# facebookresearch/PoseDiffusion

Hardware: AMD Instinct MI355X
Metric: sequences/sec (20-frame, GGS on) (higher is better)
Workload: dtype f32 (GGS, attention, LayerNorm, DDPM update, every accumulation); the encoder GEMMs multiply fp16 hi + lo operand pairs (22 bits, static power-of-two scales) with fp32 accumulation -- `exact_mode` is the same pipe with them on the exact-fp32 matrix instruction

## Files before the change

### posediffusion_amd/csrc/pd_denoiser.hip

```cpp
#include "pd_denoiser_dev.h"
#include "pd_gemm_stream.h"
#include "pd_gemm_split.h"
#include "pd_qkv_attn.h"
#ifndef PD_STRIP_RT3
#define PD_STRIP_RT3 1
#endif
#ifndef PD_STRIP_RT1
#define PD_STRIP_RT1 0
#endif
#ifndef PD_STRIP_RT3_FF1
#define PD_STRIP_RT3_FF1 0
#endif
#ifndef PD_STRIP_K64
#define PD_STRIP_K64 true
#endif

#include <algorithm>
#include <math.h>
#include <stdlib.h>
#include <string.h>

__global__ __launch_bounds__(256) void pd_embed_rows_kernel(const float *__restrict__ x, int n_frames, int M, float *__restrict__ out) {
    const int row = blockIdx.x * 4 + (threadIdx.x >> 6), lane = threadIdx.x & 63;
    if (row >= M) return;
// ... 571 lines not shown
static size_t attn_seq_lds(int N) { return ((size_t)3 * N * (DH + 4) + 4 * PD_ATTN_RPW * 64) * sizeof(float); }

struct HeadArgs {
    const float *hid;
    const float *lnw, *lnb, *w3, *b3;
    const float *x;
    const float *noise;
    float *eps_out, *mean_out, *x0_out, *xnext_out;
    float c_recip, c_recipm1, coef1, coef2, sigma;
    int M;
    int pred_x0;
#ifdef PD_DEN_STAMPS
    long long *stamps;
#endif
};

__global__ __launch_bounds__(256) void pd_tail_kernel(HeadArgs g) {
#ifdef PD_DEN_STAMPS
    long long *const stamps = g.stamps;
#endif
    PD_STAMP(stamps, 0);
    const int lane = threadIdx.x & 63, wave = threadIdx.x >> 6;
    const int m = blockIdx.x * 4 + wave;
    if (m >= g.M) return;
    const float *row = g.hid + (size_t)m * HID;
    const float v0 = row[lane], v1 = row[64 + lane];
    const int l9 = lane < 9 ? lane : 8;
    const size_t at = (size_t)m * 9 + l9;
    const float b3v = g.b3[l9], xv = g.x[at], nz = g.noise ? g.noise[at] : 0.0f;
    const float mean = pd_wave_sum(v0 + v1) * (1.0f / HID);
    const float d0 = v0 - mean, d1 = v1 - mean;
    const float rstd = 1.0f / sqrtf(pd_wave_sum(d0 * d0 + d1 * d1) * (1.0f / HID) + 1e-5f);
    const float a0 = pd_relu(d0 * rstd * g.lnw[lane] + g.lnb[lane]);
    const float a1 = pd_relu(d1 * rstd * g.lnw[64 + lane] + g.lnb[64 + lane]);
    float e = 0.0f;
#pragma unroll
    for (int o = 0; o < 9; ++o) {
        const float part = pd_wave_sum(fmaf(a0, g.w3[o * HID + lane], a1 * g.w3[o * HID + 64 + lane]));
        e = (lane == o) ? part : e;
    }
    if (lane < 9) {
        e += b3v;
        const float x0 = g.pred_x0 ? e : g.c_recip * xv - g.c_recipm1 * e;
        const float mu = g.coef1 * x0 + g.coef2 * xv;
        if (g.eps_out) g.eps_out[at] = e;
        if (g.x0_out) g.x0_out[at] = x0;
        if (g.mean_out) g.mean_out[at] = mu;
        if (g.xnext_out) g.xnext_out[at] = g.noise ? mu + g.sigma * nz : mu;
    }
    PD_STAMP(stamps, 5);
    PD_STAMP_DRAIN();
    PD_STAMP(stamps, 6);
}

int pd_time_table(const pd_weights *w, float *table) {
    if (!w->time_w0 || !w->time_b0 || !w->time_w2 || !w->time_b2) {
        pd_set_error("pd_engine_create: a weight pointer is NULL");
        return PD_ERR_INVALID_ARG;
    }
    hipLaunchKernelGGL(pd_time_table_kernel, dim3(w->timesteps), dim3(128), 0, 0, w->time_w0, w->time_b0, w->time_w2, w->time_b2, table);
    PD_HIP_CHECK(hipGetLastError());
    return PD_OK;
}

static bool pd_denoiser_default_shape(const pd_weights *w) {
    return w->d_model == DM && w->nhead == NH && w->dim_ff == DFF && w->z_dim == ZD && w->n_harmonic == 10 && w->t_emb_dim == 256 &&
           w->mlp_hidden == HID && w->num_layers >= 1 && w->num_layers <= PD_MAX_LAYERS &&
           !(w->reserved & (PD_WEIGHTS_POST_NORM | PD_WEIGHTS_NO_PIVOT | PD_WEIGHTS_GENERIC));
}

int pd_denoiser_create(pd_engine *eng, const pd_weights *w) {
    if (!pd_denoiser_default_shape(w)) return pd_denoiser_generic_create(eng, w);
    PdDenoiserDev *d = new PdDenoiserDev();
    eng->den = d;
    PdDevAllocs &m = d->mem;
    d->num_layers = w->num_layers;
    d->timesteps = w->timesteps;
    d->m_cap = ((eng->max_B * eng->max_N + 31) / 32) * 32;
    PD_TRY(m.alloc(&d->t_table, (size_t)w->timesteps * 128));
    PD_TRY(pd_time_table(w, d->t_table));
    for (int v = 0; v < 2; ++v) {
        const int nt = v ? 16 : 32;
        PD_TRY(m.pack(&d->first_wp[v], w->first_w, DM, KFIRST, KFIRST_PAD, nt, nullptr, 1));
        PD_TRY(m.pack(&d->last0_wp[v], w->last0_w, HID, DM, DM, nt, nullptr));
        for (int l = 0; l < w->num_layers; ++l) {
            const pd_layer_weights &s = w->layers[l];
            PdLayerDev &L = d->layers[l];
            PD_TRY(m.pack(&L.qkv_wp[v], s.in_proj_w, 3 * DM, DM, DM, nt, s.norm1_w));
            PD_TRY(m.pack(&L.out_wp[v], s.out_proj_w, DM, DM, DM, nt, nullptr));
            PD_TRY(m.pack(&L.ff1_wp[v], s.linear1_w, DFF, DM, DM, nt, s.norm2_w));
            PD_TRY(m.pack(&L.ff2_wp[v], s.linear2_w, DM, DFF, DFF, nt, nullptr));
        }
    }
    PD_TRY(m.copy(&d->first_b, w->first_b, DM));
    for (int l = 0; l < w->num_layers; ++l) {
        const pd_layer_weights &s = w->layers[l];
        PdLayerDev &L = d->layers[l];
        if (!s.norm1_w || !s.norm2_w) {
            pd_set_error("pd_engine_create: a LayerNorm weight pointer is NULL");
            return PD_ERR_INVALID_ARG;
        }
        PD_TRY(m.fold_bias(&L.qkv_b, s.in_proj_w, s.norm1_b, s.in_proj_b, 3 * DM, DM));
        PD_TRY(m.copy(&L.out_b, s.out_proj_b, DM));
        PD_TRY(m.fold_bias(&L.ff1_b, s.linear1_w, s.norm2_b, s.linear1_b, DFF, DM));
        PD_TRY(m.copy(&L.ff2_b, s.linear2_b, DM));
        PD_TRY(m.rowmajor(&L.qkv_wf, s.in_proj_w, 3 * DM, DM, s.norm1_w));
        PD_TRY(m.rowmajor(&L.out_wf, s.out_proj_w, DM, DM, nullptr));
        PD_TRY(m.rowmajor(&L.ff1_wf, s.linear1_w, DFF, DM, s.norm2_w));
        PD_TRY(m.rowmajor(&L.ff2_wf, s.linear2_w, DM, DFF, nullptr));
    }
    PD_TRY(m.copy(&d->last0_b, w->last0_b, HID));
    PD_TRY(m.copy(&d->last_ln_w, w->last_ln_w, HID));
    PD_TRY(m.copy(&d->last_ln_b, w->last_ln_b, HID));
    PD_TRY(m.copy(&d->last3_w, w->last3_w, 9 * HID));
    PD_TRY(m.copy(&d->last3_b, w->last3_b, 9));
    const size_t rows = (size_t)d->m_cap;
    PD_TRY(m.alloc(&d->h, rows * DM));
    PD_TRY(m.alloc(&d->qkv, rows * 3 * DM));
    PD_TRY(m.alloc(&d->ctx, rows * DM));
    PD_TRY(m.alloc(&d->ff, rows * DFF));
    PD_TRY(m.alloc(&d->hid, rows * HID));
    if (rows >= PD_STREAM_MIN_ROWS) PD_TRY(m.alloc(&d->hn, rows * DM));
    if (d->hn) {
        PD_TRY(m.alloc(&d->emb, rows * KFIRST_D));
        PD_TRY(m.alloc(&d->zproj, rows * DM));
        PD_TRY(m.alloc(&d->first_df, (size_t)DM * KFIRST_D));
        PD_TRY(m.alloc(&d->first_zf, (size_t)DM * ZD));
        hipLaunchKernelGGL(pd_first_rowmajor_kernel, dim3((DM * KFIRST_D + 255) / 256), dim3(256), 0, 0, w->first_w, d->first_df, PD_FIRST_D, KFIRST_D);
        hipLaunchKernelGGL(pd_first_rowmajor_kernel, dim3((DM * ZD + 255) / 256), dim3(256), 0, 0, w->first_w, d->first_zf, PD_FIRST_Z, ZD);
        PD_HIP_CHECK(hipGetLastError());
        PD_TRY(m.alloc(&d->ttab, (size_t)w->timesteps * DM));
        hipLaunchKernelGGL(pd_first_ttab_kernel, dim3(w->timesteps), dim3(DM), 0, 0, w->first_w, d->t_table, d->ttab);
        PD_HIP_CHECK(hipGetLastError());
    }
    PD_TRY(m.rowmajor(&d->last0_wf, w->last0_w, HID, DM, nullptr));
    PD_TRY(pd_set_lds(pd_gemm_kernel<KFIRST_PAD, 2, 0, 32>, 32 * (KFIRST_PAD + 4) * 4));
    PD_TRY(pd_set_lds(pd_gemm_kernel<KFIRST_PAD, 2, 0, 16>, 32 * (KFIRST_PAD + 4) * 4));
    PD_TRY(pd_set_lds(pd_gemm_kernel<DM, 1, 0, 32>, 32 * (DM + 4) * 4));
    PD_TRY(pd_set_lds(pd_gemm_kernel<DM, 1, 0, 16>, 32 * (DM + 4) * 4));
    PD_TRY(pd_set_lds(pd_gemm_kernel<DM, 1, 1, 32>, 32 * (DM + 4) * 4));
    PD_TRY(pd_set_lds(pd_gemm_kernel<DM, 1, 1, 16>, 32 * (DM + 4) * 4));
    PD_TRY(pd_set_lds(pd_gemm_kernel<DM, 0, 2, 32>, 32 * (DM + 4) * 4));
    PD_TRY(pd_set_lds(pd_gemm_kernel<DM, 0, 2, 16>, 32 * (DM + 4) * 4));
    PD_TRY(pd_set_lds(pd_gemm_kernel<DFF, 0, 2, 32>, 32 * (DFF + 4) * 4));
    PD_TRY(pd_set_lds(pd_gemm_kernel<DFF, 0, 2, 16>, 32 * (DFF + 4) * 4));
    PD_TRY(pd_set_lds(pd_gemm_kernel<DM, 0, 0, 32>, 32 * (DM + 4) * 4));
    PD_TRY(pd_set_lds(pd_gemm_kernel<DM, 0, 0, 16>, 32 * (DM + 4) * 4));
    PD_TRY(pd_set_lds(pd_attn_kernel<false>, ((2 * 64 + 4) * (DH + 4) + 4 * 64) * 4));
    PD_TRY(pd_set_lds(pd_attn_kernel<true>, ((2 * 64 + 4) * (DH + 4) + 4 * 64) * 4));
    PD_TRY(pd_set_lds(pd_attn_seq_kernel<0>, attn_seq_lds(64)));
    PD_TRY(pd_set_lds(pd_attn_seq_kernel<1>, attn_seq_lds(64)));
    PD_TRY(pd_set_lds(pd_attn_seq_kernel<2>, attn_seq_lds(64)));
    PD_TRY(pd_set_lds(pd_attn_mma_kernel<2>, attn_mma_lds(32)));
    PD_TRY(pd_set_lds((pd_qkv_attn_kernel<0, PD_QA_DEEP_DEFAULT != 0>), 160 * 1024));
#ifdef PD_DEV_KNOBS
    PD_TRY(pd_set_lds((pd_qkv_attn_kernel<0, PD_QA_DEEP_DEFAULT == 0>), 160 * 1024));
    PD_TRY(pd_set_lds(pd_qkv_attn_kernel<1>, 160 * 1024));
    PD_TRY(pd_set_lds(pd_qkv_attn_kernel<2>, 160 * 1024));
    PD_TRY(pd_set_lds(pd_qkv_attn_kernel<3>, 160 * 1024));
    PD_TRY(pd_set_lds(pd_qkv_attn_kernel<4>, 160 * 1024));
    PD_TRY(pd_set_lds(pd_qkv_attn_kernel<5>, 160 * 1024));
#endif
    PD_HIP_CHECK(hipDeviceSynchronize());
    return PD_OK;
}

bool pd_denoiser_has_streamed_path(const pd_engine *eng) { return eng->den && eng->den->hn; }
bool pd_denoiser_weights_non_finite(const pd_engine *eng) { return eng->den && eng->den->non_finite; }

int pd_denoiser_build_split(pd_engine *eng, int mode) {
    if (eng->gden) {
        pd_set_error("split-precision denoiser: this engine runs the shape-generic denoiser path (a non-default configuration or "
                     "PD_WEIGHTS_GENERIC), which has only the exact-fp32 kernels: PD_OPT_DENOISER_SPLIT stays 0");
        return PD_ERR_UNSUPPORTED;
    }
    PdDenoiserDev *d = eng->den;
    if (!d->hn) {
        pd_set_error("split-precision denoiser: the engine was created for fewer than %d token rows (max_B x max_N); the mode "
                     "applies to the streamed large-batch path only", PD_STREAM_MIN_ROWS);
        return PD_ERR_UNSUPPORTED;
    }
    const bool f16 = mode == 2;
    bool &ready = f16 ? d->split_h_ready : d->split_ready;
    if (ready) return PD_OK;
    PdPlaneExps e[PD_MAX_LAYERS] = {};
    for (int l = 0; f16 && l < d->num_layers; ++l) {
        PdLayerDev &L = d->layers[l];
        bool finite = true;
        PD_TRY(pd_plane_exponents(L.qkv_wf, L.qkv_b, L.out_wf, L.ff1_wf, L.ff1_b, L.ff2_wf, DM, DFF, &e[l], &finite));
        if (!finite) {
            d->non_finite = true;
            pd_set_error("denoiser: encoder layer %d holds non-finite weights or biases: no static operand bound exists, the fp16-plane "
                         "mode (PD_OPT_DENOISER_SPLIT = 2) is not available for these weights", l);
            return PD_ERR_INVALID_ARG;
        }
    }
    const int e_ln = 9;
    for (int l = 0; l < d->num_layers; ++l) {
        PdLayerDev &L = d->layers[l];
        PD_TRY(d->mem.planes(f16 ? &L.qkv_wh : &L.qkv_ws, L.qkv_wf, 3 * DM, DM, nullptr, f16, e[l].qkv));
        PD_TRY(d->mem.planes(f16 ? &L.out_wh : &L.out_ws, L.out_wf, DM, DM, nullptr, f16, e[l].out));
        PD_TRY(d->mem.planes(f16 ? &L.ff1_wh : &L.ff1_ws, L.ff1_wf, DFF, DM, nullptr, f16, e[l].ff1));
        PD_TRY(d->mem.planes(f16 ? &L.ff2_wh : &L.ff2_ws, L.ff2_wf, DM, DFF, nullptr, f16, e[l].ff2));
        if (!f16) continue;
        L.qkv_cs = ldexpf(1.0f, -(e_ln + e[l].qkv));
        L.out_cs = ldexpf(1.0f, -(e[l].ctx + e[l].out));
        L.ff1_cs = ldexpf(1.0f, -(e_ln + e[l].ff1));
        L.ff2_cs = ldexpf(1.0f, -(e[l].hid + e[l].ff2));
        L.ctx_scale = ldexpf(1.0f, e[l].ctx);
        L.ff_scale = ldexpf(1.0f, e[l].hid);
    }
    PD_HIP_CHECK(hipDeviceSynchronize());
    ready = true;
    return PD_OK;
}

void pd_denoiser_destroy(pd_engine *eng) {
    pd_denoiser_generic_destroy(eng);
    delete eng->den;
    eng->den = nullptr;
}

#ifdef PD_DEN_STAMPS
static long long *g_den_stamps = nullptr;
static int g_den_stamp_slot = 0;
#define PD_DEN_STAMP_SLOTS 256
static long long *next_stamp_slot() {
    if (!g_den_stamps) {
        if (hipMalloc((void **)&g_den_stamps, sizeof(long long) * 8 * PD_DEN_STAMP_SLOTS) != hipSuccess) return nullptr;
        (void)hipMemset(g_den_stamps, 0, sizeof(long long) * 8 * PD_DEN_STAMP_SLOTS);
    }
    long long *p = g_den_stamps + 8 * (g_den_stamp_slot % PD_DEN_STAMP_SLOTS);
    g_den_stamp_slot += 1;
    return p;
}
extern "C" int pd_debug_den_stamps(long long *out, int n_slots) {
    if (!out || n_slots <= 0 || n_slots > PD_DEN_STAMP_SLOTS || !g_den_stamps) return PD_ERR_INVALID_ARG;
    PD_HIP_CHECK(hipDeviceSynchronize());
    PD_HIP_CHECK(hipMemcpy(out, g_den_stamps, sizeof(long long) * 8 * n_slots, hipMemcpyDeviceToHost));
    PD_HIP_CHECK(hipMemset(g_den_stamps, 0, sizeof(long long) * 8 * PD_DEN_STAMP_SLOTS));
    g_den_stamp_slot = 0;
    return PD_OK;
}
#endif
template <int K, int AMODE, int EPI>
static void launch_gemm(GemmArgs &g, float *const wp[2], int MT, int wide_min, hipStream_t s) {
    const int tiles32 = MT * (g.Nout / 32);
    g.MT = MT;
#ifdef PD_DEN_STAMPS
    g.stamps = next_stamp_slot();
#endif
    if (tiles32 >= wide_min && (g.Nout / 32) % 8 == 0) {
        g.Wp = wp[0];
        hipLaunchKernelGGL((pd_gemm_kernel<K, AMODE, EPI, 32>), dim3(MT * (g.Nout / 32)), dim3(256), 32 * (K + 4) * 4, s, g);
    } else {
        g.Wp = wp[1];
        hipLaunchKernelGGL((pd_gemm_kernel<K, AMODE, EPI, 16>), dim3(MT * (g.Nout / 16)), dim3(256), 32 * (K + 4) * 4, s, g);
    }
}

int pd_denoiser_prepare(pd_engine *eng, const float *z, int B, int N, hipStream_t s) {
    PdDenoiserDev *d = eng->den;
    if (eng->gden) d = nullptr;
    if (!z || B <= 0 || N <= 0 || B > eng->max_B || N > eng->max_N) {
        pd_set_error("denoiser: invalid arguments (B=%d N=%d; max_B=%d max_N=%d)", B, N, eng->max_B, eng->max_N);
        return PD_ERR_INVALID_ARG;
    }
    if (!d) return PD_OK;
    const int M = B * N;
    if (M >= PD_STREAM_MIN_ROWS && d->hn) pd_gemm_dma<0>(z, ZD, d->first_zf, ZD, d->first_b, d->zproj, M, DM, s);
    PD_HIP_CHECK(hipGetLastError());
    return PD_OK;
}

int pd_denoiser_launch(pd_engine *eng, const float *x, const float *z, int t, int B, int N, float *eps_out,
                       float *mean_out, float *x0_out, const float *noise, float *x_next_out, hipStream_t s, bool z_prepared) {
    if (eng->gden) return pd_denoiser_generic_launch(eng, x, z, t, B, N, eps_out, mean_out, x0_out, noise, x_next_out, s);
    PdDenoiserDev *d = eng->den;
    if (!x || !z || B <= 0 || N <= 0 || B > eng->max_B || N > eng->max_N || N > 64 || t < 0 || t >= d->timesteps) {
        pd_set_error("denoiser: invalid arguments (B=%d N=%d t=%d; max_B=%d max_N=%d, N <= 64, 0 <= t < %d)", B, N, t,
                     eng->max_B, eng->max_N, d->timesteps);
        return PD_ERR_INVALID_ARG;
    }
    if (!z_prepared) {
        int rc = pd_denoiser_prepare(eng, z, B, N, s);
        if (rc) return rc;
    }
    const int M = B * N, MT = (M + 31) / 32;
    GemmArgs g;
    memset(&g, 0, sizeof(g));
    g.M = M;
    const bool streamed = M >= PD_STREAM_MIN_ROWS && d->hn;
    if (streamed) {
        hipLaunchKernelGGL(pd_embed_rows_kernel, dim3((M + 3) / 4), dim3(256), 0, s, x, N, M, d->emb);
        pd_gemm_dma<4>(d->emb, KFIRST_D, d->first_df, KFIRST_D, d->ttab + (size_t)t * DM, d->h, M, DM, s, nullptr, d->zproj);
    } else {
        g.bias = d->first_b; g.C = d->h; g.Nout = DM;
        g.x = x; g.z = z; g.temb = d->t_table + (size_t)t * 128; g.n_frames = N;
        launch_gemm<KFIRST_PAD, 2, 0>(g, d->first_wp, MT, eng->gemm_wide_min_tiles, s);
    }
    for (int l = 0; l < d->num_layers; ++l) {
        const PdLayerDev &L = d->layers[l];
        if (streamed && eng->den_split == 2 && d->split_h_ready) {
            static const int strip = pd_dev_knob("PD_DEN_STRIP", 15);
            hipLaunchKernelGGL((pd_ln_rows_kernel<DM, 2>), dim3((M + 3) / 4), dim3(256), 0, s, d->h, d->hn, M, 1e-5f, 512.0f);
            static const int attn_mma = pd_dev_knob("PD_DEN_ATTN_MMA", 1);
            const int qa_wgs = ((B + pd_qkv_attn_group(N > 32 ? 1 : N) - 1) / pd_qkv_attn_group(N > 32 ? 1 : N)) * NH, cus = eng->num_cus > 0 ? eng->num_cus : 256;
            const bool qa_fills = 4 * qa_wgs >= 3 * ((qa_wgs + cus - 1) / cus) * cus;
            if (N <= 32 && eng->den_fused_attn == 1 ? qa_fills : (N <= 32 && eng->den_fused_attn == 2)) {
                pd_qkv_attn((const unsigned *)d->hn, L.qkv_wh, L.qkv_b, (unsigned *)d->ctx, B, N, L.qkv_cs, L.ctx_scale, s);
            } else {
                if (strip & 1) pd_gemm_strip<0, 2, true, 1, PD_STRIP_K64>((const unsigned *)d->hn, DM, L.qkv_wh, DM, L.qkv_b, d->qkv, M, 3 * DM, s, L.qkv_cs);
                else pd_gemm_split<0, 1, 2, true>((const unsigned *)d->hn, DM, L.qkv_wh, DM, L.qkv_b, d->qkv, M, 3 * DM, s, L.qkv_cs);
                if (N <= 32 && attn_mma) hipLaunchKernelGGL(pd_attn_mma_kernel<2>, dim3(B * NH), dim3(256), attn_mma_lds(N), s, d->qkv, d->ctx, N, L.ctx_scale);
// ... 149 lines not shown
```

### posediffusion_amd/csrc/pd_qkv_attn.h

```cpp
#pragma once
#include "pd_gemm_split.h"

#ifndef PD_QA_XCD_MAP
#define PD_QA_XCD_MAP 1
#endif
#define PD_QA_WAVES 12
#define PD_QA_THREADS (PD_QA_WAVES * 64)
#define PD_QA_ROWS 96
#define PD_QA_LDR (3 * DH + 4)
#define PD_QA_LS 36
#ifndef PD_QA_DEEP_DEFAULT
#define PD_QA_DEEP_DEFAULT 0
#endif

struct PdQkvAttnArgs {
    const unsigned *A;
    const unsigned *W;
    const float *bias;
    unsigned *ctx;
    int B, N, G;
    float c_scale, out_scale;
};
static inline int pd_qkv_attn_group(int N) { return N >= 1 && N <= 32 ? (PD_QA_ROWS - 1) / N : 0; }
static inline size_t pd_qkv_attn_lds(int N) {
    const int G = pd_qkv_attn_group(N);
    const size_t image = (size_t)(G * N + 1) * PD_QA_LDR * sizeof(float);
    const size_t stage = (size_t)4 * PD_QA_ROWS * 32 * sizeof(unsigned);
    return (image > stage ? image : stage) + (size_t)3 * 32 * PD_QA_LS * sizeof(float);
}

template <int BARE, bool DEEP = false>
__global__ __launch_bounds__(PD_QA_THREADS) void pd_qkv_attn_kernel(PdQkvAttnArgs g) {
    constexpr int KC = 32, RT = 3, TM = PD_QA_ROWS, CHA = TM * KC, LDR = PD_QA_LDR, LS = PD_QA_LS;
    extern __shared__ __attribute__((aligned(1024))) unsigned qa_lds[];
    const int tid = threadIdx.x, lane = tid & 63, l31 = lane & 31, hi = lane >> 5;
    const int wave = __builtin_amdgcn_readfirstlane(tid >> 6);
    int head = blockIdx.x & 3, grp = blockIdx.x >> 2;
#if PD_QA_XCD_MAP == 1
    {
        const int ngrp = gridDim.x >> 2, c = blockIdx.x >> 4, r = blockIdx.x & 15;
        if (4 * c + 4 <= ngrp) {
            head = 2 * ((r & 7) >> 2) + (r >> 3);
            grp = 4 * c + (r & 3);
        }
    }
#elif PD_QA_XCD_MAP == 2
    {
        const int ngrp = gridDim.x >> 2, c = blockIdx.x >> 5, r = blockIdx.x & 31;
        if (8 * c + 8 <= ngrp) {
            head = r >> 3;
            grp = 8 * c + (r & 7);
        }
    }
#endif
    const int N = g.N, G = g.G, M = g.B * N;
    const int seq0 = grp * G, nseq = min(G, g.B - seq0), m0 = seq0 * N, rows = nseq * N;
    const int prow = lane >> 3, pslot = lane & 7;
    unsigned oa;
    {
        const int r = 8 * wave + prow;
        oa = (unsigned)(((size_t)min(m0 + r, M - 1) * DM + 4 * (pslot ^ ((r >> 1) & 7))) * sizeof(unsigned));
    }
    const unsigned lds_a = (unsigned)(size_t)(qa_lds + wave * 256);
    const int third = wave >> 2;
    const int ntile = third * (DM / 32) + head * (DH / 32) + (wave & 3);
    constexpr int KS = DM / 16;
    const uint4 *wq = (const uint4 *)g.W + (size_t)ntile * KS * 128 + lane;
    typedef unsigned wv4 __attribute__((ext_vector_type(4)));
    f32x16 acc[RT];
#pragma unroll
    for (int mi = 0; mi < RT; ++mi)
#pragma unroll
        for (int i = 0; i < 16; ++i) acc[mi][i] = 0.0f;
    auto mmaw = [](const uint4 &a, const wv4 &b, const f32x16 &c) {
        return __builtin_amdgcn_mfma_f32_32x32x16_f16(__builtin_bit_cast(f16x8, a), __builtin_bit_cast(f16x8, b), c, 0, 0, 0);
    };
#define PD_QA_WLOAD(w0, w1, w2, w3, b)                                                                                               \
    do {                                                                                                                             \
        const uint4 *wp_ = wq + (size_t)(b) * 256;                                                                                   \
        asm volatile("global_load_dwordx4 %0, %4, off\n\tglobal_load_dwordx4 %1, %4, off offset:1024\n\t"                           \
                     "global_load_dwordx4 %2, %4, off offset:2048\n\tglobal_load_dwordx4 %3, %4, off offset:3072"                    \
                     : "=&v"(w0), "=&v"(w1), "=&v"(w2), "=&v"(w3) : "v"(wp_) : "memory");                                            \
    } while (0)
#define PD_QA_WAIT(n, w0, w1, w2, w3) asm volatile("s_waitcnt vmcnt(" #n ")" : "+v"(w0), "+v"(w1), "+v"(w2), "+v"(w3) : : "memory")
    auto stage64 = [&](int c, int buf) {
        const unsigned da = __builtin_amdgcn_readfirstlane(lds_a + buf * 2 * CHA * 4);
#pragma unroll
        for (int h = 0; h < 2; ++h) pd_dma_piece((const float *)(g.A + (2 * c + h) * KC), oa, da + h * CHA * 4);
    };
    auto block = [&](const unsigned *a, const wv4 &w0, const wv4 &w1, const wv4 &w2, const wv4 &w3) {
        uint4 ah[RT], al[RT];
#pragma unroll
        for (int st = 0; st < 2; ++st) {
#pragma unroll
            for (int mi = 0; mi < RT; ++mi) {
                const uint4 p = *(const uint4 *)(a + mi * 32 * KC + 4 * ((4 * st + 2 * hi) ^ ((l31 >> 1) & 7)));
                const uint4 q = *(const uint4 *)(a + mi * 32 * KC + 4 * ((4 * st + 2 * hi + 1) ^ ((l31 >> 1) & 7)));
                ah[mi] = make_uint4(__builtin_amdgcn_perm(p.y, p.x, 0x05040100u), __builtin_amdgcn_perm(p.w, p.z, 0x05040100u),
                                    __builtin_amdgcn_perm(q.y, q.x, 0x05040100u), __builtin_amdgcn_perm(q.w, q.z, 0x05040100u));
                al[mi] = make_uint4(__builtin_amdgcn_perm(p.y, p.x, 0x07060302u), __builtin_amdgcn_perm(p.w, p.z, 0x07060302u),
                                    __builtin_amdgcn_perm(q.y, q.x, 0x07060302u), __builtin_amdgcn_perm(q.w, q.z, 0x07060302u));
            }
            const wv4 &wh = st ? w2 : w0, &wl = st ? w3 : w1;
#pragma unroll
            for (int mi = 0; mi < RT; ++mi) acc[mi] = mmaw(al[mi], wh, acc[mi]);
#pragma unroll
            for (int mi = 0; mi < RT; ++mi) acc[mi] = mmaw(ah[mi], wl, acc[mi]);
#pragma unroll
            for (int mi = 0; mi < RT; ++mi) acc[mi] = mmaw(ah[mi], wh, acc[mi]);
        }
    };
    {
        wv4 a0, a1, a2, a3, b0, b1, b2, b3;
        constexpr int nk64 = DM / 64;
        stage64(0, 0);
        PD_QA_WLOAD(a0, a1, a2, a3, 0);
        PD_QA_WLOAD(b0, b1, b2, b3, 1);
        PD_QA_WAIT(0, a0, a1, a2, a3);
        PD_QA_WAIT(0, b0, b1, b2, b3);
        __syncthreads();
        if constexpr (DEEP) {
            static_assert(!DEEP || BARE == 0, "the deep form has no development variants");
            wv4 c0, c1, c2, c3, d0, d1, d2, d3;
            for (int c = 0; c < nk64; c += 2) {
                {
                    const unsigned *a = qa_lds + 0 * 2 * CHA + l31 * KC;
                    stage64(c + 1, 1);
                    PD_QA_WLOAD(c0, c1, c2, c3, 2 * (c + 1));
                    PD_QA_WLOAD(d0, d1, d2, d3, 2 * (c + 1) + 1);
                    block(a, a0, a1, a2, a3);
                    block(a + CHA, b0, b1, b2, b3);
                    PD_QA_WAIT(0, c0, c1, c2, c3);
                    PD_QA_WAIT(0, d0, d1, d2, d3);
                    __syncthreads();
                }
                {
                    const int cn = min(c + 2, nk64 - 1);
                    const unsigned *a = qa_lds + 1 * 2 * CHA + l31 * KC;
                    stage64(cn, 0);
                    PD_QA_WLOAD(a0, a1, a2, a3, 2 * cn);
                    PD_QA_WLOAD(b0, b1, b2, b3, 2 * cn + 1);
                    block(a, c0, c1, c2, c3);
                    block(a + CHA, d0, d1, d2, d3);
                    PD_QA_WAIT(0, a0, a1, a2, a3);
                    PD_QA_WAIT(0, b0, b1, b2, b3);
                    __syncthreads();
                }
            }
        } else
        for (int c = 0; c < nk64; ++c) {
            const int cn = min(c + 1, nk64 - 1);
            const unsigned *a = qa_lds + (c & 1) * 2 * CHA + l31 * KC;
            if constexpr (BARE == 0) {
                if (c + 1 < nk64) {
                    stage64(cn, (c + 1) & 1);
                    block(a, a0, a1, a2, a3);
                    PD_QA_WLOAD(a0, a1, a2, a3, 2 * cn);
                    PD_QA_WAIT(6, b0, b1, b2, b3);
                    block(a + CHA, b0, b1, b2, b3);
                    PD_QA_WLOAD(b0, b1, b2, b3, 2 * cn + 1);
                    PD_QA_WAIT(4, a0, a1, a2, a3);
                } else {
                    block(a, a0, a1, a2, a3);
                    PD_QA_WAIT(0, b0, b1, b2, b3);
                    block(a + CHA, b0, b1, b2, b3);
                }
            } else {
                if constexpr (BARE != 2 && BARE != 3) stage64(cn, (c + 1) & 1);
                if constexpr (BARE != 4) block(a, a0, a1, a2, a3);
                if constexpr (BARE != 1 && BARE != 3) PD_QA_WLOAD(a0, a1, a2, a3, 2 * cn);
                if constexpr (BARE != 4) block(a + CHA, b0, b1, b2, b3);
                if constexpr (BARE != 1 && BARE != 3) PD_QA_WLOAD(b0, b1, b2, b3, 2 * cn + 1);
                PD_QA_WAIT(0, a0, a1, a2, a3);
                PD_QA_WAIT(0, b0, b1, b2, b3);
            }
            __syncthreads();
        }
        PD_QA_WAIT(0, b0, b1, b2, b3);
    }
#undef PD_QA_WLOAD
#undef PD_QA_WAIT
    if constexpr (BARE == 5) {
        if (acc[0][0] == 123.456f) g.ctx[tid] = 1u;
        return;
    }
    float *img = (float *)qa_lds;
    float *Sall = img + (size_t)(G * N + 1) * LDR;
    {
        const int col = ntile * 32 + l31;
        const float bias = g.bias[col];
        const int lcol = third * DH + (wave & 3) * 32 + l31;
        const float qscale = 0.08838834764831845f;
#pragma unroll
        for (int mi = 0; mi < RT; ++mi)
#pragma unroll
            for (int i = 0; i < 16; ++i) {
                const int row = mi * 32 + 4 * hi + (i & 3) + 8 * (i >> 2);
                float v = fmaf(acc[mi][i], g.c_scale, bias);
                if (third == 0) v *= qscale;
                if (row < rows) img[row * LDR + lcol] = v;
            }
        for (int c = tid; c < LDR; c += PD_QA_THREADS) img[G * N * LDR + c] = 0.0f;
    }
    __syncthreads();
    const int team = wave >> 2, tw = wave & 3, ttid = tid & 255;
    float *S = Sall + team * 32 * LS;
    const int rounds = (G + 2) / 3;
    for (int rd = 0; rd < rounds; ++rd) {
        const int s = rd * 3 + team;
        const bool active = s < nseq;
        const float *base = img + (size_t)s * N * LDR;
        const float *zrow = img + (size_t)G * N * LDR;
        auto rowp = [&](int j) { return j < N ? base + j * LDR : zrow; };
        if (active) {
            const float *qa = rowp(16 * (tw >> 1) + (lane & 15)) + 4 * (lane >> 4);
            const float *kb = rowp(16 * (tw & 1) + (lane & 15)) + DH + 4 * (lane >> 4);
            f32x4 sc = {0.f, 0.f, 0.f, 0.f};
#pragma unroll
            for (int c = 0; c < DH / 16; ++c) {
                const float4 a = *(const float4 *)(qa + 16 * c), k = *(const float4 *)(kb + 16 * c);
                sc = __builtin_amdgcn_mfma_f32_16x16x4f32(a.x, k.x, sc, 0, 0, 0);
                sc = __builtin_amdgcn_mfma_f32_16x16x4f32(a.y, k.y, sc, 0, 0, 0);
                sc = __builtin_amdgcn_mfma_f32_16x16x4f32(a.z, k.z, sc, 0, 0, 0);
                sc = __builtin_amdgcn_mfma_f32_16x16x4f32(a.w, k.w, sc, 0, 0, 0);
            }
            const int j = 16 * (tw & 1) + (lane & 15);
#pragma unroll
            for (int e = 0; e < 4; ++e) S[(16 * (tw >> 1) + 4 * (lane >> 4) + e) * LS + j] = sc[e];
        }
        __syncthreads();
        if (active) {
            const int i = ttid >> 3, sub = ttid & 7;
            float4 sv = *(const float4 *)(S + i * LS + 4 * sub);
            const int j0 = 4 * sub;
            sv.x = j0 + 0 < N ? sv.x : -INFINITY;
            sv.y = j0 + 1 < N ? sv.y : -INFINITY;
            sv.z = j0 + 2 < N ? sv.z : -INFINITY;
            sv.w = j0 + 3 < N ? sv.w : -INFINITY;
            float mx = fmaxf(fmaxf(sv.x, sv.y), fmaxf(sv.z, sv.w));
            mx = fmaxf(mx, __shfl_xor(mx, 1, 64));
            mx = fmaxf(mx, __shfl_xor(mx, 2, 64));
            mx = fmaxf(mx, __shfl_xor(mx, 4, 64));
            float4 e;
            e.x = j0 + 0 < N ? expf(sv.x - mx) : 0.0f;
            e.y = j0 + 1 < N ? expf(sv.y - mx) : 0.0f;
            e.z = j0 + 2 < N ? expf(sv.z - mx) : 0.0f;
            e.w = j0 + 3 < N ? expf(sv.w - mx) : 0.0f;
            const float inv = 1.0f / pd_sum8((e.x + e.y) + (e.z + e.w));
            e.x *= inv; e.y *= inv; e.z *= inv; e.w *= inv;
            *(float4 *)(S + i * LS + 4 * sub) = e;
        }
        __syncthreads();
        if (active) {
            f32x4 o[2][2];
#pragma unroll
            for (int rt = 0; rt < 2; ++rt)
#pragma unroll
                for (int ct = 0; ct < 2; ++ct) o[rt][ct] = f32x4{0.f, 0.f, 0.f, 0.f};
            const float *pa = S + (lane & 15) * LS + 4 * (lane >> 4);
            const int vcol = 2 * DH + 32 * tw + (lane & 15);
            const int jg = 4 * (lane >> 4);
#pragma unroll
            for (int c = 0; c < 2; ++c) {
                const float4 p0 = *(const float4 *)(pa + 16 * c), p1 = *(const float4 *)(pa + 16 * LS + 16 * c);
                float v0[4], v1[4];
#pragma unroll
                for (int e = 0; e < 4; ++e) {
                    const float *vr = rowp(16 * c + jg + e) + vcol;
                    v0[e] = vr[0];
                    v1[e] = vr[16];
                }
                const float a0[4] = {p0.x, p0.y, p0.z, p0.w}, a1[4] = {p1.x, p1.y, p1.z, p1.w};
#pragma unroll
                for (int e = 0; e < 4; ++e) {
                    o[0][0] = __builtin_amdgcn_mfma_f32_16x16x4f32(a0[e], v0[e], o[0][0], 0, 0, 0);
                    o[0][1] = __builtin_amdgcn_mfma_f32_16x16x4f32(a0[e], v1[e], o[0][1], 0, 0, 0);
                    o[1][0] = __builtin_amdgcn_mfma_f32_16x16x4f32(a1[e], v0[e], o[1][0], 0, 0, 0);
                    o[1][1] = __builtin_amdgcn_mfma_f32_16x16x4f32(a1[e], v1[e], o[1][1], 0, 0, 0);
                }
            }
#pragma unroll
            for (int rt = 0; rt < 2; ++rt)
#pragma unroll
                for (int e = 0; e < 4; ++e) {
                    const int i = 16 * rt + 4 * (lane >> 4) + e;
                    if (i < N) {
                        unsigned *out = g.ctx + (size_t)((seq0 + s) * N + i) * DM + head * DH + 32 * tw + (lane & 15);
#pragma unroll
                        for (int ct = 0; ct < 2; ++ct) out[16 * ct] = pd_split_word_as<2>(o[rt][ct][e], g.out_scale);
                    }
                }
        }
        __syncthreads();
    }
}

static inline void pd_qkv_attn(const unsigned *hn, const unsigned *Wh, const float *bias, unsigned *ctx, int B, int N, float c_scale, float out_scale,
                               hipStream_t s) {
    const int G = pd_qkv_attn_group(N);
    PdQkvAttnArgs g{hn, Wh, bias, ctx, B, N, G, c_scale, out_scale};
#ifdef PD_DEV_KNOBS
    static const int bare = pd_dev_knob("PD_QA_BARE", 0);
    const dim3 grid(((B + G - 1) / G) * NH), blk(PD_QA_THREADS);
    const size_t lds = pd_qkv_attn_lds(N);
    static const int deep = pd_dev_knob("PD_QA_DEEP", PD_QA_DEEP_DEFAULT);
    if (bare == 0 && !deep) { hipLaunchKernelGGL((pd_qkv_attn_kernel<0, false>), grid, blk, lds, s, g); return; }
    switch (bare) {
    case 1: hipLaunchKernelGGL(pd_qkv_attn_kernel<1>, grid, blk, lds, s, g); return;
    case 2: hipLaunchKernelGGL(pd_qkv_attn_kernel<2>, grid, blk, lds, s, g); return;
    case 3: hipLaunchKernelGGL(pd_qkv_attn_kernel<3>, grid, blk, lds, s, g); return;
    case 4: hipLaunchKernelGGL(pd_qkv_attn_kernel<4>, grid, blk, lds, s, g); return;
    case 5: hipLaunchKernelGGL(pd_qkv_attn_kernel<5>, grid, blk, lds, s, g); return;
    default: break;
    }
#endif
    hipLaunchKernelGGL((pd_qkv_attn_kernel<0, PD_QA_DEEP_DEFAULT != 0>), dim3(((B + G - 1) / G) * NH), dim3(PD_QA_THREADS), pd_qkv_attn_lds(N), s, g);
}
```

Before: 1111.

## Stage 128-wide K chunks and batch two sequences per team in fused QKV-attention

The fused QKV+attention kernel now stages A in 128-wide K chunks (four 32-k blocks) per double-buffer step instead of 64, which halves the barriers in the projection loop and lengthens the weight-load prefetch chain. The attention phase processes up to two sequences per team per round, interleaving their MFMAs to improve ILP and cutting rounds and syncs. Context output is first written into the LDS image and then copied out as coalesced uint4 stores. The unused DEEP variant is dropped. The cost is more LDS for staging and scores, and more registers.

```diff
diff --git a/posediffusion_amd/csrc/pd_denoiser.hip b/posediffusion_amd/csrc/pd_denoiser.hip
--- a/posediffusion_amd/csrc/pd_denoiser.hip
+++ b/posediffusion_amd/csrc/pd_denoiser.hip
@@ -747,14 +747,13 @@
     PD_TRY(pd_set_lds(pd_attn_seq_kernel<1>, attn_seq_lds(64)));
     PD_TRY(pd_set_lds(pd_attn_seq_kernel<2>, attn_seq_lds(64)));
     PD_TRY(pd_set_lds(pd_attn_mma_kernel<2>, attn_mma_lds(32)));
-    PD_TRY(pd_set_lds((pd_qkv_attn_kernel<0, PD_QA_DEEP_DEFAULT != 0>), 160 * 1024));
+    PD_TRY(pd_set_lds(pd_qkv_attn_kernel<0>, PD_QA_LDS_MAX));
 #ifdef PD_DEV_KNOBS
-    PD_TRY(pd_set_lds((pd_qkv_attn_kernel<0, PD_QA_DEEP_DEFAULT == 0>), 160 * 1024));
-    PD_TRY(pd_set_lds(pd_qkv_attn_kernel<1>, 160 * 1024));
-    PD_TRY(pd_set_lds(pd_qkv_attn_kernel<2>, 160 * 1024));
-    PD_TRY(pd_set_lds(pd_qkv_attn_kernel<3>, 160 * 1024));
-    PD_TRY(pd_set_lds(pd_qkv_attn_kernel<4>, 160 * 1024));
-    PD_TRY(pd_set_lds(pd_qkv_attn_kernel<5>, 160 * 1024));
+    PD_TRY(pd_set_lds(pd_qkv_attn_kernel<1>, PD_QA_LDS_MAX));
+    PD_TRY(pd_set_lds(pd_qkv_attn_kernel<2>, PD_QA_LDS_MAX));
+    PD_TRY(pd_set_lds(pd_qkv_attn_kernel<3>, PD_QA_LDS_MAX));
+    PD_TRY(pd_set_lds(pd_qkv_attn_kernel<4>, PD_QA_LDS_MAX));
+    PD_TRY(pd_set_lds(pd_qkv_attn_kernel<5>, PD_QA_LDS_MAX));
 #endif
     PD_HIP_CHECK(hipDeviceSynchronize());
     return PD_OK;
diff --git a/posediffusion_amd/csrc/pd_qkv_attn.h b/posediffusion_amd/csrc/pd_qkv_attn.h
--- a/posediffusion_amd/csrc/pd_qkv_attn.h
+++ b/posediffusion_amd/csrc/pd_qkv_attn.h
@@ -1,4 +1,5 @@
 #pragma once
+#include <type_traits>
 #include "pd_gemm_split.h"
 
 #ifndef PD_QA_XCD_MAP
@@ -9,29 +10,42 @@
 #define PD_QA_ROWS 96
 #define PD_QA_LDR (3 * DH + 4)
 #define PD_QA_LS 36
-#ifndef PD_QA_DEEP_DEFAULT
-#define PD_QA_DEEP_DEFAULT 0
-#endif
+#define PD_QA_KB 4
+#define PD_QA_QMAX 2
+#define PD_QA_LDS_MAX (160 * 1024)
 
 struct PdQkvAttnArgs {
     const unsigned *A;
     const unsigned *W;
     const float *bias;
     unsigned *ctx;
-    int B, N, G;
+    int B, N, G, Q;
     float c_scale, out_scale;
 };
-static inline int pd_qkv_attn_group(int N) { return N >= 1 && N <= 32 ? (PD_QA_ROWS - 1) / N : 0; }
-static inline size_t pd_qkv_attn_lds(int N) {
-    const int G = pd_qkv_attn_group(N);
-    const size_t image = (size_t)(G * N + 1) * PD_QA_LDR * sizeof(float);
-    const size_t stage = (size_t)4 * PD_QA_ROWS * 32 * sizeof(unsigned);
-    return (image > stage ? image : stage) + (size_t)3 * 32 * PD_QA_LS * sizeof(float);
-}
+static constexpr int pd_qkv_attn_group(int N) { return N >= 1 && N <= 32 ? (PD_QA_ROWS - 1) / N : 0; }
+static constexpr size_t pd_qkv_attn_lds_base(int N) {
+    const size_t image = (size_t)(pd_qkv_attn_group(N) * N + 1) * PD_QA_LDR * sizeof(float);
+    const size_t stage = (size_t)2 * PD_QA_KB * PD_QA_ROWS * 32 * sizeof(unsigned);
+    return image > stage ? image : stage;
+}
+static constexpr size_t pd_qkv_attn_tile() { return (size_t)32 * PD_QA_LS * sizeof(float); }
+static constexpr int pd_qkv_attn_q(int N) {
+    int q = (pd_qkv_attn_group(N) + 2) / 3;
+    if (q > PD_QA_QMAX) q = PD_QA_QMAX;
+    while (q > 1 && pd_qkv_attn_lds_base(N) + 3 * q * pd_qkv_attn_tile() > PD_QA_LDS_MAX) --q;
+    return q < 1 ? 1 : q;
+}
+static constexpr size_t pd_qkv_attn_lds(int N) { return pd_qkv_attn_lds_base(N) + 3 * pd_qkv_attn_q(N) * pd_qkv_attn_tile(); }
+static constexpr bool pd_qkv_attn_lds_fits() {
+    for (int N = 1; N <= 32; ++N)
+        if (pd_qkv_attn_lds(N) > PD_QA_LDS_MAX) return false;
+    return true;
+}
+static_assert(pd_qkv_attn_lds_fits(), "image + score tiles within the 160 KiB of LDS for every N <= 32");
 
-template <int BARE, bool DEEP = false>
+template <int BARE>
 __global__ __launch_bounds__(PD_QA_THREADS) void pd_qkv_attn_kernel(PdQkvAttnArgs g) {
-    constexpr int KC = 32, RT = 3, TM = PD_QA_ROWS, CHA = TM * KC, LDR = PD_QA_LDR, LS = PD_QA_LS;
+    constexpr int KC = 32, RT = 3, TM = PD_QA_ROWS, CHA = TM * KC, KB = PD_QA_KB, LDR = PD_QA_LDR, LS = PD_QA_LS;
     extern __shared__ __attribute__((aligned(1024))) unsigned qa_lds[];
     const int tid = threadIdx.x, lane = tid & 63, l31 = lane & 31, hi = lane >> 5;
     const int wave = __builtin_amdgcn_readfirstlane(tid >> 6);
@@ -83,10 +97,10 @@
                      : "=&v"(w0), "=&v"(w1), "=&v"(w2), "=&v"(w3) : "v"(wp_) : "memory");                                            \
     } while (0)
 #define PD_QA_WAIT(n, w0, w1, w2, w3) asm volatile("s_waitcnt vmcnt(" #n ")" : "+v"(w0), "+v"(w1), "+v"(w2), "+v"(w3) : : "memory")
-    auto stage64 = [&](int c, int buf) {
-        const unsigned da = __builtin_amdgcn_readfirstlane(lds_a + buf * 2 * CHA * 4);
-#pragma unroll
-        for (int h = 0; h < 2; ++h) pd_dma_piece((const float *)(g.A + (2 * c + h) * KC), oa, da + h * CHA * 4);
+    auto stage128 = [&](int c, int buf) {
+        const unsigned da = __builtin_amdgcn_readfirstlane(lds_a + buf * KB * CHA * 4);
+#pragma unroll
+        for (int h = 0; h < KB; ++h) pd_dma_piece((const float *)(g.A + (KB * c + h) * KC), oa, da + h * CHA * 4);
     };
     auto block = [&](const unsigned *a, const wv4 &w0, const wv4 &w1, const wv4 &w2, const wv4 &w3) {
         uint4 ah[RT], al[RT];
@@ -112,70 +126,63 @@
     };
     {
         wv4 a0, a1, a2, a3, b0, b1, b2, b3;
-        constexpr int nk64 = DM / 64;
-        stage64(0, 0);
+        constexpr int nk128 = DM / (KB * KC), nblk = DM / KC;
+        static_assert(DM % (KB * KC) == 0 && nk128 >= 2, "whole 128-k chunks");
+        stage128(0, 0);
         PD_QA_WLOAD(a0, a1, a2, a3, 0);
         PD_QA_WLOAD(b0, b1, b2, b3, 1);
         PD_QA_WAIT(0, a0, a1, a2, a3);
         PD_QA_WAIT(0, b0, b1, b2, b3);
         __syncthreads();
-        if constexpr (DEEP) {
-            static_assert(!DEEP || BARE == 0, "the deep form has no development variants");
-            wv4 c0, c1, c2, c3, d0, d1, d2, d3;
-            for (int c = 0; c < nk64; c += 2) {
-                {
-                    const unsigned *a = qa_lds + 0 * 2 * CHA + l31 * KC;
-                    stage64(c + 1, 1);
-                    PD_QA_WLOAD(c0, c1, c2, c3, 2 * (c + 1));
-                    PD_QA_WLOAD(d0, d1, d2, d3, 2 * (c + 1) + 1);
+        auto chunk = [&](int c, auto last_) {
+            constexpr bool LAST = decltype(last_)::value;
+            const unsigned *a = qa_lds + (c & 1) * KB * CHA + l31 * KC;
+            const int b0i = KB * c;
+            if constexpr (BARE == 0) {
+                if constexpr (!LAST) {
+                    stage128(c + 1, (c + 1) & 1);
                     block(a, a0, a1, a2, a3);
+                    PD_QA_WLOAD(a0, a1, a2, a3, b0i + 2);
+                    PD_QA_WAIT(8, b0, b1, b2, b3);
                     block(a + CHA, b0, b1, b2, b3);
-                    PD_QA_WAIT(0, c0, c1, c2, c3);
-                    PD_QA_WAIT(0, d0, d1, d2, d3);
-                    __syncthreads();
-                }
-                {
-                    const int cn = min(c + 2, nk64 - 1);
-                    const unsigned *a = qa_lds + 1 * 2 * CHA + l31 * KC;
-                    stage64(cn, 0);
-                    PD_QA_WLOAD(a0, a1, a2, a3, 2 * cn);
-                    PD_QA_WLOAD(b0, b1, b2, b3, 2 * cn + 1);
-                    block(a, c0, c1, c2, c3);
-                    block(a + CHA, d0, d1, d2, d3);
-                    PD_QA_WAIT(0, a0, a1, a2, a3);
-                    PD_QA_WAIT(0, b0, b1, b2, b3);
-                    __syncthreads();
-                }
-            }
-        } else
-        for (int c = 0; c < nk64; ++c) {
-            const int cn = min(c + 1, nk64 - 1);
-            const unsigned *a = qa_lds + (c & 1) * 2 * CHA + l31 * KC;
-            if constexpr (BARE == 0) {
-                if (c + 1 < nk64) {
-                    stage64(cn, (c + 1) & 1);
-                    block(a, a0, a1, a2, a3);
-                    PD_QA_WLOAD(a0, a1, a2, a3, 2 * cn);
-                    PD_QA_WAIT(6, b0, b1, b2, b3);
-                    block(a + CHA, b0, b1, b2, b3);
-                    PD_QA_WLOAD(b0, b1, b2, b3, 2 * cn + 1);
+                    PD_QA_WLOAD(b0, b1, b2, b3, b0i + 3);
+                    PD_QA_WAIT(4, a0, a1, a2, a3);
+                    block(a + 2 * CHA, a0, a1, a2, a3);
+                    PD_QA_WLOAD(a0, a1, a2, a3, b0i + 4);
+                    PD_QA_WAIT(4, b0, b1, b2, b3);
+                    block(a + 3 * CHA, b0, b1, b2, b3);
+                    PD_QA_WLOAD(b0, b1, b2, b3, b0i + 5);
                     PD_QA_WAIT(4, a0, a1, a2, a3);
                 } else {
                     block(a, a0, a1, a2, a3);
+                    PD_QA_WLOAD(a0, a1, a2, a3, b0i + 2);
+                    PD_QA_WAIT(4, b0, b1, b2, b3);
+                    block(a + CHA, b0, b1, b2, b3);
+                    PD_QA_WLOAD(b0, b1, b2, b3, b0i + 3);
+                    PD_QA_WAIT(4, a0, a1, a2, a3);
+                    block(a + 2 * CHA, a0, a1, a2, a3);
                     PD_QA_WAIT(0, b0, b1, b2, b3);
-                    block(a + CHA, b0, b1, b2, b3);
+                    block(a + 3 * CHA, b0, b1, b2, b3);
                 }
             } else {
-                if constexpr (BARE != 2 && BARE != 3) stage64(cn, (c + 1) & 1);
+                if constexpr (!LAST && BARE != 2 && BARE != 3) stage128(c + 1, (c + 1) & 1);
                 if constexpr (BARE != 4) block(a, a0, a1, a2, a3);
-                if constexpr (BARE != 1 && BARE != 3) PD_QA_WLOAD(a0, a1, a2, a3, 2 * cn);
+                if constexpr (BARE != 1 && BARE != 3) PD_QA_WLOAD(a0, a1, a2, a3, b0i + 2);
                 if constexpr (BARE != 4) block(a + CHA, b0, b1, b2, b3);
-                if constexpr (BARE != 1 && BARE != 3) PD_QA_WLOAD(b0, b1, b2, b3, 2 * cn + 1);
+                if constexpr (BARE != 1 && BARE != 3) PD_QA_WLOAD(b0, b1, b2, b3, b0i + 3);
                 PD_QA_WAIT(0, a0, a1, a2, a3);
                 PD_QA_WAIT(0, b0, b1, b2, b3);
+                if constexpr (BARE != 4) block(a + 2 * CHA, a0, a1, a2, a3);
+                if constexpr (BARE != 1 && BARE != 3) PD_QA_WLOAD(a0, a1, a2, a3, min(b0i + 4, nblk - 2));
+                if constexpr (BARE != 4) block(a + 3 * CHA, b0, b1, b2, b3);
+                if constexpr (BARE != 1 && BARE != 3) PD_QA_WLOAD(b0, b1, b2, b3, min(b0i + 5, nblk - 1));
+                PD_QA_WAIT(0, a0, a1, a2, a3);
+                PD_QA_WAIT(0, b0, b1, b2, b3);
             }
             __syncthreads();
-        }
+        };
+        for (int c = 0; c + 1 < nk128; ++c) chunk(c, std::false_type{});
+        chunk(nk128 - 1, std::true_type{});
         PD_QA_WAIT(0, b0, b1, b2, b3);
     }
 #undef PD_QA_WLOAD
@@ -204,34 +211,51 @@
     }
     __syncthreads();
     const int team = wave >> 2, tw = wave & 3, ttid = tid & 255;
-    float *S = Sall + team * 32 * LS;
-    const int rounds = (G + 2) / 3;
+    const int Q = g.Q;
+    float *S = Sall + team * Q * 32 * LS;
+    const float *zrow = img + (size_t)G * N * LDR;
+    auto rowp = [&](int s, int j) { return j < N ? img + ((size_t)s * N + j) * LDR : zrow; };
+    const int rounds = (nseq + 3 * Q - 1) / (3 * Q);
     for (int rd = 0; rd < rounds; ++rd) {
-        const int s = rd * 3 + team;
-        const bool active = s < nseq;
-        const float *base = img + (size_t)s * N * LDR;
-        const float *zrow = img + (size_t)G * N * LDR;
-        auto rowp = [&](int j) { return j < N ? base + j * LDR : zrow; };
-        if (active) {
-            const float *qa = rowp(16 * (tw >> 1) + (lane & 15)) + 4 * (lane >> 4);
-            const float *kb = rowp(16 * (tw & 1) + (lane & 15)) + DH + 4 * (lane >> 4);
-            f32x4 sc = {0.f, 0.f, 0.f, 0.f};
+        const int s0 = rd * 3 * Q + team;
+        const int nq = s0 >= nseq ? 0 : (Q > 1 && s0 + 3 < nseq ? 2 : 1);
+        auto scores = [&](auto nq_) {
+            constexpr int NQ = decltype(nq_)::value;
+            const float *qa[NQ], *kb[NQ];
+            f32x4 sc[NQ];
+#pragma unroll
+            for (int u = 0; u < NQ; ++u) {
+                qa[u] = rowp(s0 + 3 * u, 16 * (tw >> 1) + (lane & 15)) + 4 * (lane >> 4);
+                kb[u] = rowp(s0 + 3 * u, 16 * (tw & 1) + (lane & 15)) + DH + 4 * (lane >> 4);
+                sc[u] = f32x4{0.f, 0.f, 0.f, 0.f};
+            }
 #pragma unroll
             for (int c = 0; c < DH / 16; ++c) {
-                const float4 a = *(const float4 *)(qa + 16 * c), k = *(const float4 *)(kb + 16 * c);
-                sc = __builtin_amdgcn_mfma_f32_16x16x4f32(a.x, k.x, sc, 0, 0, 0);
-                sc = __builtin_amdgcn_mfma_f32_16x16x4f32(a.y, k.y, sc, 0, 0, 0);
-                sc = __builtin_amdgcn_mfma_f32_16x16x4f32(a.z, k.z, sc, 0, 0, 0);
-                sc = __builtin_amdgcn_mfma_f32_16x16x4f32(a.w, k.w, sc, 0, 0, 0);
+                float4 a[NQ], k[NQ];
+#pragma unroll
+                for (int u = 0; u < NQ; ++u) a[u] = *(const float4 *)(qa[u] + 16 * c), k[u] = *(const float4 *)(kb[u] + 16 * c);
+#pragma unroll
+                for (int u = 0; u < NQ; ++u) sc[u] = __builtin_amdgcn_mfma_f32_16x16x4f32(a[u].x, k[u].x, sc[u], 0, 0, 0);
+#pragma unroll
+                for (int u = 0; u < NQ; ++u) sc[u] = __builtin_amdgcn_mfma_f32_16x16x4f32(a[u].y, k[u].y, sc[u], 0, 0, 0);
+#pragma unroll
+                for (int u = 0; u < NQ; ++u) sc[u] = __builtin_amdgcn_mfma_f32_16x16x4f32(a[u].z, k[u].z, sc[u], 0, 0, 0);
+#pragma unroll
+                for (int u = 0; u < NQ; ++u) sc[u] = __builtin_amdgcn_mfma_f32_16x16x4f32(a[u].w, k[u].w, sc[u], 0, 0, 0);
             }
             const int j = 16 * (tw & 1) + (lane & 15);
 #pragma unroll
-            for (int e = 0; e < 4; ++e) S[(16 * (tw >> 1) + 4 * (lane >> 4) + e) * LS + j] = sc[e];
-        }
+            for (int u = 0; u < NQ; ++u)
+#pragma unroll
+                for (int e = 0; e < 4; ++e) S[u * 32 * LS + (16 * (tw >> 1) + 4 * (lane >> 4) + e) * LS + j] = sc[u][e];
+        };
+        if (nq == 2) scores(std::integral_constant<int, 2>{});
+        else if (nq == 1) scores(std::integral_constant<int, 1>{});
         __syncthreads();
-        if (active) {
+        for (int u = 0; u < nq; ++u) {
+            float *Su = S + u * 32 * LS;
             const int i = ttid >> 3, sub = ttid & 7;
-            float4 sv = *(const float4 *)(S + i * LS + 4 * sub);
+            float4 sv = *(const float4 *)(Su + i * LS + 4 * sub);
             const int j0 = 4 * sub;
             sv.x = j0 + 0 < N ? sv.x : -INFINITY;
             sv.y = j0 + 1 < N ? sv.y : -INFINITY;
@@ -248,63 +272,88 @@
             e.w = j0 + 3 < N ? expf(sv.w - mx) : 0.0f;
             const float inv = 1.0f / pd_sum8((e.x + e.y) + (e.z + e.w));
             e.x *= inv; e.y *= inv; e.z *= inv; e.w *= inv;
-            *(float4 *)(S + i * LS + 4 * sub) = e;
+            *(float4 *)(Su + i * LS + 4 * sub) = e;
         }
         __syncthreads();
-        if (active) {
-            f32x4 o[2][2];
-#pragma unroll
-            for (int rt = 0; rt < 2; ++rt)
-#pragma unroll
-                for (int ct = 0; ct < 2; ++ct) o[rt][ct] = f32x4{0.f, 0.f, 0.f, 0.f};
+        auto pv = [&](auto nq_) {
+            constexpr int NQ = decltype(nq_)::value;
+            f32x4 o[NQ][2][2];
+#pragma unroll
+            for (int u = 0; u < NQ; ++u)
+#pragma unroll
+                for (int rt = 0; rt < 2; ++rt)
+#pragma unroll
+                    for (int ct = 0; ct < 2; ++ct) o[u][rt][ct] = f32x4{0.f, 0.f, 0.f, 0.f};
             const float *pa = S + (lane & 15) * LS + 4 * (lane >> 4);
             const int vcol = 2 * DH + 32 * tw + (lane & 15);
             const int jg = 4 * (lane >> 4);
 #pragma unroll
             for (int c = 0; c < 2; ++c) {
-                const float4 p0 = *(const float4 *)(pa + 16 * c), p1 = *(const float4 *)(pa + 16 * LS + 16 * c);
-                float v0[4], v1[4];
-#pragma unroll
-                for (int e = 0; e < 4; ++e) {
-                    const float *vr = rowp(16 * c + jg + e) + vcol;
-                    v0[e] = vr[0];
-                    v1[e] = vr[16];
-                }
-                const float a0[4] = {p0.x, p0.y, p0.z, p0.w}, a1[4] = {p1.x, p1.y, p1.z, p1.w};
-#pragma unroll
-                for (int e = 0; e < 4; ++e) {
-                    o[0][0] = __builtin_amdgcn_mfma_f32_16x16x4f32(a0[e], v0[e], o[0][0], 0, 0, 0);
-                    o[0][1] = __builtin_amdgcn_mfma_f32_16x16x4f32(a0[e], v1[e], o[0][1], 0, 0, 0);
-                    o[1][0] = __builtin_amdgcn_mfma_f32_16x16x4f32(a1[e], v0[e], o[1][0], 0, 0, 0);
-                    o[1][1] = __builtin_amdgcn_mfma_f32_16x16x4f32(a1[e], v1[e], o[1][1], 0, 0, 0);
-                }
-            }
-#pragma unroll
-            for (int rt = 0; rt < 2; ++rt)
-#pragma unroll
-                for (int e = 0; e < 4; ++e) {
-                    const int i = 16 * rt + 4 * (lane >> 4) + e;
-                    if (i < N) {
-                        unsigned *out = g.ctx + (size_t)((seq0 + s) * N + i) * DM + head * DH + 32 * tw + (lane & 15);
-#pragma unroll
-                        for (int ct = 0; ct < 2; ++ct) out[16 * ct] = pd_split_word_as<2>(o[rt][ct][e], g.out_scale);
+                float a0[NQ][4], a1[NQ][4], v0[NQ][4], v1[NQ][4];
+#pragma unroll
+                for (int u = 0; u < NQ; ++u) {
+                    const float4 p0 = *(const float4 *)(pa + u * 32 * LS + 16 * c), p1 = *(const float4 *)(pa + u * 32 * LS + 16 * LS + 16 * c);
+                    a0[u][0] = p0.x, a0[u][1] = p0.y, a0[u][2] = p0.z, a0[u][3] = p0.w;
+                    a1[u][0] = p1.x, a1[u][1] = p1.y, a1[u][2] = p1.z, a1[u][3] = p1.w;
+#pragma unroll
+                    for (int e = 0; e < 4; ++e) {
+                        const float *vr = rowp(s0 + 3 * u, 16 * c + jg + e) + vcol;
+                        v0[u][e] = vr[0];
+                        v1[u][e] = vr[16];
                     }
                 }
-        }
-        __syncthreads();
+#pragma unroll
+                for (int e = 0; e < 4; ++e)
+#pragma unroll
+                    for (int u = 0; u < NQ; ++u) {
+                        o[u][0][0] = __builtin_amdgcn_mfma_f32_16x16x4f32(a0[u][e], v0[u][e], o[u][0][0], 0, 0, 0);
+                        o[u][0][1] = __builtin_amdgcn_mfma_f32_16x16x4f32(a0[u][e], v1[u][e], o[u][0][1], 0, 0, 0);
+                        o[u][1][0] = __builtin_amdgcn_mfma_f32_16x16x4f32(a1[u][e], v0[u][e], o[u][1][0], 0, 0, 0);
+                        o[u][1][1] = __builtin_amdgcn_mfma_f32_16x16x4f32(a1[u][e], v1[u][e], o[u][1][1], 0, 0, 0);
+                    }
+            }
+#pragma unroll
+            for (int u = 0; u < NQ; ++u) {
+                const int s = s0 + 3 * u;
+                unsigned *tq = (unsigned *)(img + (size_t)s * N * LDR) + 32 * tw;
+#pragma unroll
+                for (int rt = 0; rt < 2; ++rt)
+#pragma unroll
+                    for (int e = 0; e < 4; ++e) {
+                        const int i = 16 * rt + 4 * (lane >> 4) + e;
+                        if (i < N) {
+#pragma unroll
+                            for (int ct = 0; ct < 2; ++ct) tq[i * LDR + 16 * ct + (lane & 15)] = pd_split_word_as<2>(o[u][rt][ct][e], g.out_scale);
+                        }
+                    }
+            }
+            asm volatile("s_waitcnt lgkmcnt(0)" : : : "memory");
+#pragma unroll
+            for (int u = 0; u < NQ; ++u) {
+                const int s = s0 + 3 * u;
+                const unsigned *tq = (const unsigned *)(img + (size_t)s * N * LDR) + 32 * tw;
+                unsigned *out = g.ctx + (size_t)(seq0 + s) * N * DM + head * DH + 32 * tw;
+#pragma unroll
+                for (int it = 0; it < 4; ++it) {
+                    const int i = 8 * it + (lane >> 3), c4 = 4 * (lane & 7);
+                    if (i < N) *(uint4 *)(out + (size_t)i * DM + c4) = *(const uint4 *)(tq + i * LDR + c4);
+                }
+            }
+        };
+        if (nq == 2) pv(std::integral_constant<int, 2>{});
+        else if (nq == 1) pv(std::integral_constant<int, 1>{});
+        if (rd + 1 < rounds) __syncthreads();
     }
 }
 
 static inline void pd_qkv_attn(const unsigned *hn, const unsigned *Wh, const float *bias, unsigned *ctx, int B, int N, float c_scale, float out_scale,
                                hipStream_t s) {
     const int G = pd_qkv_attn_group(N);
-    PdQkvAttnArgs g{hn, Wh, bias, ctx, B, N, G, c_scale, out_scale};
+    PdQkvAttnArgs g{hn, Wh, bias, ctx, B, N, G, pd_qkv_attn_q(N), c_scale, out_scale};
+    const dim3 grid(((B + G - 1) / G) * NH), blk(PD_QA_THREADS);
+    const size_t lds = pd_qkv_attn_lds(N);
 #ifdef PD_DEV_KNOBS
     static const int bare = pd_dev_knob("PD_QA_BARE", 0);
-    const dim3 grid(((B + G - 1) / G) * NH), blk(PD_QA_THREADS);
-    const size_t lds = pd_qkv_attn_lds(N);
-    static const int deep = pd_dev_knob("PD_QA_DEEP", PD_QA_DEEP_DEFAULT);
-    if (bare == 0 && !deep) { hipLaunchKernelGGL((pd_qkv_attn_kernel<0, false>), grid, blk, lds, s, g); return; }
     switch (bare) {
     case 1: hipLaunchKernelGGL(pd_qkv_attn_kernel<1>, grid, blk, lds, s, g); return;
     case 2: hipLaunchKernelGGL(pd_qkv_attn_kernel<2>, grid, blk, lds, s, g); return;
@@ -314,5 +363,5 @@
     default: break;
     }
 #endif
-    hipLaunchKernelGGL((pd_qkv_attn_kernel<0, PD_QA_DEEP_DEFAULT != 0>), dim3(((B + G - 1) / G) * NH), dim3(PD_QA_THREADS), pd_qkv_attn_lds(N), s, g);
-}
+    hipLaunchKernelGGL(pd_qkv_attn_kernel<0>, grid, blk, lds, s, g);
+}
```

After: 1095. -1.5%, worse.
